# VGLoic/kzg-poly-commit-exploration

Hardware: AMD Instinct MI355X
Metric: g1_msm_commitments_per_sec_degree_2^20 (higher is better)
Workload: dtype i32 digits (Fp: 13 signed radix-2^30 digits, Montgomery 2^390; Fr: 8 x u32, Montgomery 2^256)

## Files before the change

kzg_poly_commit_exploration_amd/csrc/api.hip:

```cpp
#include <hip/hip_runtime.h>
#include <sys/random.h>

#include <algorithm>
#include <atomic>
#include <cerrno>
#include <chrono>
#include <condition_variable>
#include <cstdio>
#include <cstdlib>
#include <cstring>
#include <deque>
#include <functional>
#include <mutex>
#include <new>
#include <string>
#include <thread>
#include <vector>

#include "../../include/kzg_mi355x.h"
#include "engine.h"
#include "host_field.hpp"
#include "host_fr.hpp"
#include "fr30_host.hpp"
#include "host_pairing.hpp"
// ... 91 lines not shown
        DevBuf& b = buf[i];
        int rc = KZG_OK;
        if (!bytes && !b.p) {
            rc = b.reserve(ctx, 256);
            b.cap = 0;
        } else {
            rc = b.reserve(ctx, bytes);
        }
        *out = b.p;
        return rc;
    }
};

struct SlotQueue {
    hipStream_t stream = nullptr;
    hipStream_t end = nullptr;
    hipEvent_t ev[8] = {};
    hipEvent_t done = nullptr;
    hipEvent_t sorted_ev = nullptr, accum_ev = nullptr;
    hipEvent_t cmb_ev[2] = {};
    hipEvent_t cells_ev = nullptr;
    hipEvent_t upload_ev = nullptr;
    SlotQueue() = default;
    SlotQueue(const SlotQueue&) = delete;
    SlotQueue& operator=(const SlotQueue&) = delete;
    ~SlotQueue() {
        for (hipEvent_t e : {ev[0], ev[1], ev[2], ev[3], ev[4], ev[5], ev[6], ev[7], cmb_ev[0], cmb_ev[1], cells_ev, upload_ev, done, sorted_ev, accum_ev})
            if (e) hipEventDestroy(e);
    }
};

struct Slot : SlotQueue {
    DevBuf cnt, offs, block_sums, pairs, sorted, buckets;
    DevBuf part_a, part_b;
    DevBuf pair_scratch;
    DevBuf heavy_ws;
    DevBuf arena;
    PinnedBuf fin{PinnedBuf::Mapped};
    DevBuf stage;
    DevBuf q;
    DevBuf chunk, block;
    PinnedBuf small{PinnedBuf::Mapped};
    PinnedBuf bsmall{PinnedBuf::Mapped};
    std::vector<uint32_t> open_ys;
    PinnedBuf roots{PinnedBuf::Staged};
    PinnedBuf pvals{PinnedBuf::Mapped};
    DevBuf pblock;
    std::vector<uint32_t> pts_ys;
    size_t pts_nq = 0;
    PinnedBuf ctab{PinnedBuf::Staged};
    PinnedBuf cvals{PinnedBuf::Mapped};
    DevBuf cpart, cin;
    size_t cmb_t = 0;
    float combine_ms = 0;
    PinnedBuf stab{PinnedBuf::Staged}, ssel{PinnedBuf::Staged};
    PinnedBuf svals{PinnedBuf::Mapped};
    DevBuf sg;
    std::vector<uint32_t> sets_vmap;
    DevBuf lag_part;
    DevBuf gp_in, gp_z, gp_part;
    PinnedBuf gp_flags{PinnedBuf::Mapped};
    DevBuf cpoly, cagg;
    SlotKind kind = SLOT_IDLE;
    size_t job_n = 0;
    uint32_t job_batch = 1;
    uint32_t open_y[8] = {};
// ... 60 lines not shown
        if (_e != hipSuccess) {                                                                     \
            (ctx)->last_error = std::string(#expr) + ": " + hipGetErrorString(_e);                  \
            return KZG_ERR_HIP;                                                                     \
        }                                                                                           \
    } while (0)

int hip_fail(kzg_ctx* ctx, const char* what, hipError_t e) {
    ctx->last_error = std::string(what) + ": " + hipGetErrorString(e);
    return KZG_ERR_HIP;
}

struct TmpStream {
    hipStream_t s = nullptr;
    ~TmpStream() { if (s) hipStreamDestroy(s); }
};

int sync_unlocked(kzg_ctx* ctx, std::unique_lock<std::mutex>& lk, hipStream_t st, const char* what) {
    lk.unlock();
    const hipError_t e = hipStreamSynchronize(st);
    lk.lock();
    return e == hipSuccess ? KZG_OK : hip_fail(ctx, what, e);
}
constexpr const char* kCopyCoeffs = "hipMemcpyAsync (coefficients)";
int copy_unlocked(kzg_ctx* ctx, std::unique_lock<std::mutex>& lk, hipStream_t st, void* dst, const void* src, size_t bytes,
                  hipMemcpyKind kind, const char* what) {
    if (!bytes) return KZG_OK;
    lk.unlock();
    const hipError_t e = hipMemcpyAsync(dst, src, bytes, kind, st);
    lk.lock();
    return e == hipSuccess ? KZG_OK : hip_fail(ctx, what, e);
}

void free_slot_msm(Slot& s) {
    for (DevBuf* b : {&s.cnt, &s.offs, &s.block_sums, &s.pairs, &s.sorted, &s.buckets, &s.part_a, &s.part_b, &s.pair_scratch,
                      &s.heavy_ws, &s.arena})
        b->reset();
    s.fin.reset();
}

int create_stream(kzg_ctx* ctx, hipStream_t* out, bool high) {
    int least = 0, greatest = 0;
    HIP_TRY(ctx, hipDeviceGetStreamPriorityRange(&least, &greatest));
    const char* v = std::getenv("KZG_STREAM_PRIORITIES");
    const bool prio = !(v && v[0] == '0');
    HIP_TRY(ctx, hipStreamCreateWithPriority(out, hipStreamNonBlocking, prio ? (high ? greatest : least) : 0));
    return KZG_OK;
}

int ensure_slot_basics(kzg_ctx* ctx, Slot& s) {
    if (s.stream) return KZG_OK;
    if (!ctx->front_stream) {
        int rc = create_stream(ctx, &ctx->front_stream, false);
        if (rc) return rc;
    }
    if (!ctx->upload_stream) HIP_TRY(ctx, hipStreamCreateWithFlags(&ctx->upload_stream, hipStreamNonBlocking));
    for (auto& e : s.ev)
        if (!e) HIP_TRY(ctx, hipEventCreate(&e));
    if (!s.upload_ev) HIP_TRY(ctx, hipEventCreateWithFlags(&s.upload_ev, hipEventDisableTiming));
    s.stream = s.end = ctx->front_stream;
    if (!s.done) HIP_TRY(ctx, hipEventCreateWithFlags(&s.done, hipEventDisableTiming));
    return s.small.reserve(ctx, 64 * 4);
}

int upload_unlocked(kzg_ctx* ctx, std::unique_lock<std::mutex>& lk, Slot& s, void* dst, const void* src, size_t bytes) {
    if (!bytes) return KZG_OK;
    int rc = copy_unlocked(ctx, lk, ctx->upload_stream, dst, src, bytes, hipMemcpyHostToDevice, kCopyCoeffs);
    if (rc) return rc;
// ... 60 lines not shown
            ctx->last_error = "injected allocation failure (KZG_TEST_FAIL_SLOT_ALLOC)";
            return KZG_ERR_HIP;
        }
    }
    if (!ctx->heavy_stream) {
        int rc = create_stream(ctx, &ctx->heavy_stream, true);
        if (rc) return rc;
    }
    if (!ctx->tail_stream) {
        int rc = create_stream(ctx, &ctx->tail_stream, false);
        if (rc) return rc;
    }
    const MsmConfig cfg = ctx->cfg;
    if (ctx->max_batch > sort_max_batch(cfg)) ctx->max_batch = sort_max_batch(cfg);
    const size_t B = ctx->max_batch;
    const size_t pairs = (size_t)cfg.max_digits * ctx->n * B;
    for (int i = 0; i < kNumSlots; i++) {
        Slot& s = ctx->slots[i];
        {
            int rcb = ensure_slot_basics(ctx, s);
            if (rcb) return rcb;
        }
        if (!s.sorted_ev) {
            HIP_TRY(ctx, hipEventCreateWithFlags(&s.sorted_ev, hipEventDisableTiming));
            HIP_TRY(ctx, hipEventCreateWithFlags(&s.accum_ev, hipEventDisableTiming));
        }
        free_slot_msm(s);
        int rc = s.cnt.reserve(ctx, (size_t)sort_count_entries((uint32_t)B, cfg) * 4 + 64);
        if (rc == KZG_OK) rc = s.offs.reserve(ctx, ((size_t)cfg.nb * B + 1) * 4);
        if (rc == KZG_OK) rc = s.block_sums.reserve(ctx, (size_t)sort_workspace_words() * 4);
        if (rc) return rc;
        HIP_TRY(ctx, hipMemset(s.block_sums.p, 0, (size_t)sort_workspace_zero_words() * 4));
        rc = s.pairs.reserve(ctx, (pairs ? pairs : 1) * 8);
        if (rc == KZG_OK) rc = s.sorted.reserve(ctx, (pairs ? pairs : 1) * 4);
        if (rc == KZG_OK) rc = s.buckets.reserve(ctx, (size_t)cfg.nb * B * kXyzzBytes);
        if (rc == KZG_OK) rc = s.part_a.reserve(ctx, (size_t)kMaxAccumLanes * kXyzzBytes);
        if (rc == KZG_OK) rc = s.part_b.reserve(ctx, (size_t)kMaxAccumLanes * kXyzzBytes);
        if (rc == KZG_OK) rc = s.pair_scratch.reserve(ctx, accumulate_pair_scratch_bytes(pairs));
        if (rc == KZG_OK) rc = s.heavy_ws.reserve(ctx, heavy_workspace_bytes());
        if (rc == KZG_OK) rc = s.arena.reserve(ctx, ctx->arena_records * B * kXyzzBytes);
        if (rc == KZG_OK) rc = s.fin.reserve(ctx, ctx->final_records * B * kXyzzBytes);
        if (rc) return rc;
        s.kind = SLOT_IDLE;
    }
    ctx->slots_ready = true;
    return KZG_OK;
}

int build_tables(kzg_ctx* ctx, hipStream_t st, void* d_xyzz_tmp, void* d_prefix) {
    const size_t n = ctx->n;
    for (uint32_t j = 1; j < ctx->cfg.W; j++) {
        char* prev = (char*)ctx->table.p + (size_t)(j - 1) * n * kAffineBytes;
        char* next = (char*)ctx->table.p + (size_t)j * n * kAffineBytes;
        launch_table_window(st, prev, (uint32_t)n, ctx->cfg.level_bits, d_xyzz_tmp, d_prefix, next);
    }
    HIP_TRY(ctx, hipGetLastError());
    HIP_TRY(ctx, hipStreamSynchronize(st));
    return KZG_OK;
}

int drain_all(kzg_ctx* ctx) {
    for (hipStream_t st : {ctx->upload_stream, ctx->front_stream, ctx->heavy_stream, ctx->tail_stream})
        if (st) HIP_TRY(ctx, hipStreamSynchronize(st));
    return KZG_OK;
}

// ... 10 lines not shown
    ctx->srs_gen++;
    ctx->n = 0;
    return KZG_OK;
}

int srs_prepare(kzg_ctx* ctx, size_t n) {
    if (n == 0 || n > 0x7fffffffu / 32) return KZG_ERR_INVALID_ARG;
    int rc = srs_release(ctx);
    if (rc) return rc;
    size_t free_b = 0, total_b = 0;
    HIP_TRY(ctx, hipMemGetInfo(&free_b, &total_b));
    size_t budget = (size_t)((double)free_b * 0.6);
    if (const char* v = std::getenv("KZG_TABLE_GB")) budget = (size_t)(std::strtod(v, nullptr) * 1073741824.0);
    MsmConfig cfg = choose_msm_config(n, budget);
    if ((size_t)cfg.W * n >= 0x80000000ull) return KZG_ERR_INVALID_ARG;
    ctx->cfg = cfg;
    return ctx->table.reserve(ctx, (size_t)cfg.W * n * kAffineBytes);
}

struct MsmBasis {
    const void* table;
    uint32_t stride;
};
int enqueue_msm(kzg_ctx* ctx, Slot& s, const uint32_t* d_scalars, int is_mont, size_t n, int ev_base,
                uint32_t batch = 1, uint64_t stride = 0, const MsmBasis* basis = nullptr) {
    const MsmConfig cfg = ctx->cfg;
    const void* table = basis ? basis->table : ctx->table.p;
    const uint32_t table_stride = basis ? basis->stride : (uint32_t)ctx->n;
    const uint32_t nbt = cfg.nb * batch;
    hipStream_t st = s.stream;
    s.end = st;
    if (s.timing) HIP_TRY(ctx, hipEventRecord(s.ev[ev_base], st));
    const bool header_zeroed = launch_bucket_sort(st, d_scalars, is_mont, (uint32_t)n, batch, stride, table_stride, cfg, s.cnt.dev(),
                       s.block_sums.dev(), s.pairs.dev<uint64_t>(), s.offs.dev(), s.sorted.dev(), (uint32_t*)s.heavy_ws.p);
    if (s.timing) {
        HIP_TRY(ctx, hipEventRecord(s.ev[ev_base + 1], st));
        HIP_TRY(ctx, hipEventRecord(s.ev[ev_base + 2], st));
    }
    bool alone = true;
    for (const auto& other : ctx->slots) alone = alone && (&other == &s || other.kind == SLOT_IDLE);
    const uint64_t max_refs = (uint64_t)n * cfg.max_digits * batch;
    const uint32_t lanes = accumulate_lanes(max_refs, alone);
    const ReducePlan& P = ctx->plan;
    const uint32_t R = 1u << P.hi_bits, C = 1u << P.lo_bits, B = batch;
    char* row = (char*)s.arena.p;
    char* col = row + (size_t)R * B * kXyzzBytes;
    char* fin = (char*)s.fin.d;
    const uint32_t rl = 1u << P.row_lo, rh = 1u << P.row_hi, cl = 1u << P.col_lo, ch = 1u << P.col_hi;
    const TreeSumDesc stage1[2] = {
        {s.buckets.p, row, B * R, C, C, 1, B * R, 0},
        {s.buckets.p, col, B * C, R, 1, C, C, (uint64_t)cfg.nb}};
    const TreeSumDesc stage2[4] = {
        {row, fin + (size_t)P.off_r2row * B * kXyzzBytes, B * rh, rl, rl, 1, rh, R},
        {row, fin + (size_t)P.off_c2row * B * kXyzzBytes, B * rl, rh, 1, rl, rl, R},
        {col, fin + (size_t)P.off_r2col * B * kXyzzBytes, B * ch, cl, cl, 1, ch, C},
        {col, fin + (size_t)P.off_c2col * B * kXyzzBytes, B * cl, ch, 1, cl, cl, C}};
    if (!header_zeroed) HIP_TRY(ctx, hipMemsetAsync(s.heavy_ws.p, 0, kHeavyHeaderBytes, st));
    if (max_refs <= kTinyRefs && !ctx->small_msm_off) {
        if (s.timing) HIP_TRY(ctx, hipEventRecord(s.ev[ev_base + 3], st));
        launch_small_msm(st, table, s.sorted.dev(), s.offs.dev(), nbt, lanes, max_refs, s.buckets.p, s.part_a.p, s.part_b.p,
                         s.heavy_ws.p, s.small.dev() + 26, stage1, stage2, ctx->small_lds_bytes);
        if (s.timing) HIP_TRY(ctx, hipEventRecord(s.ev[ev_base + 4], st));
    } else {
        const bool hand_over = !alone;
        hipStream_t hs = hand_over ? ctx->heavy_stream : st;
        if (hand_over) {
            HIP_TRY(ctx, hipEventRecord(s.sorted_ev, st));
// ... 6658 lines not shown
```

kzg_poly_commit_exploration_amd/csrc/engine.h:

```cpp
#pragma once
#include <hip/hip_runtime.h>
#include <stddef.h>
#include <stdint.h>

namespace kzg {

constexpr size_t kAffineBytes = 128;
constexpr size_t kAffineU4 = kAffineBytes / 16;
constexpr size_t kXyzzBytes = 256;
constexpr size_t kXyzzU4 = kXyzzBytes / 16;
constexpr size_t kXyzzWords64 = kXyzzBytes / 8;

enum : uint32_t { kRecodeWindows = 0, kRecodeNaf = 1 };
struct MsmConfig {
    uint32_t recode;
    uint32_t c;
    uint32_t W;
    uint32_t level_bits;
    uint32_t nb;
    uint32_t max_digits;
};

MsmConfig choose_msm_config(size_t n_points, size_t table_budget_bytes);

constexpr uint32_t kTinyRefs = 65536;
__host__ __device__ inline uint32_t accumulate_min_seg(uint64_t refs) { return refs <= kTinyRefs ? 4u : 8u; }
__host__ __device__ inline uint32_t accumulate_seg_len(uint32_t M, uint32_t lanes) {
    uint32_t L = (M + lanes - 1) / lanes;
    const uint32_t lo = accumulate_min_seg(M);
    return L < lo ? lo : L;
}

constexpr size_t kHeavyHeaderBytes = 1024;
uint32_t sort_count_entries(uint32_t max_batch, MsmConfig cfg);
uint32_t sort_max_batch(MsmConfig cfg);
uint32_t sort_workspace_words();
uint32_t sort_workspace_zero_words();
bool launch_bucket_sort(hipStream_t s, const uint32_t* d_scalars, int scalars_are_mont, uint32_t n, uint32_t batch,
                        uint64_t stride, uint32_t table_stride, MsmConfig cfg, uint32_t* d_cnt,
                        uint32_t* d_ws, uint64_t* d_pairs, uint32_t* d_offs, uint32_t* d_sorted, uint32_t* d_header);
constexpr uint32_t kMaxAccumLanes = 262144 + 64;
uint32_t accumulate_lanes(uint64_t max_refs, bool alone = false);
size_t accumulate_pair_scratch_bytes(uint64_t max_refs);
void launch_bucket_accumulate(hipStream_t s, const void* d_table, const uint32_t* d_sorted, const uint32_t* d_offs,
                              uint32_t nb, uint32_t lanes, void* d_buckets ,
                              void* d_part_a, void* d_part_b, uint32_t lds_reserve_bytes, void* d_pair_scratch,
                              uint64_t max_refs, void* d_clock = nullptr );
constexpr size_t kAccumClockOffset = 768;
size_t heavy_workspace_bytes();
void launch_bucket_finalize(hipStream_t s, const uint32_t* d_offs, uint32_t nb, uint32_t lanes, const void* d_part_a,
                            const void* d_part_b, void* d_buckets, void* d_heavy_ws,
                            uint32_t* d_refs_out , uint32_t group = 1);
uint32_t finalize_group_size(uint32_t nb);
struct TreeSumDesc;
uint32_t small_msm_lds_bytes();
const void* small_msm_kernel();
void launch_small_msm(hipStream_t s, const void* d_table, const uint32_t* d_sorted, const uint32_t* d_offs, uint32_t nb,
                      uint32_t lanes, uint64_t max_refs, void* d_buckets, void* d_part_a, void* d_part_b, void* d_heavy_ws,
                      uint32_t* d_refs_out, const TreeSumDesc* stage1 , const TreeSumDesc* stage2 ,
                      uint32_t lds_bytes);
struct TreeSumDesc {
    const void* in;
    void* out;
    uint32_t groups, len;
    uint64_t gstride, estride;
    uint32_t inner;
    uint64_t ostride;
};
void launch_tree_sums(hipStream_t s, const TreeSumDesc* descs, uint32_t count, bool dense = false, bool alone = true);
void launch_tree_sums_two_stage(hipStream_t s, const TreeSumDesc* stage1, uint32_t count1, const TreeSumDesc* stage2,
                                uint32_t count2, uint32_t* d_sync, bool alone);

void launch_jacobian_to_affine(hipStream_t s, const void* d_jac, uint32_t n, void* d_affine_out,
// ... 257 lines not shown
```

kzg_poly_commit_exploration_amd/csrc/msm_sort.hip:

```cpp
#include <cstdlib>
#include <cstring>

#include "engine.h"
#include "fr30.hip.h"

namespace kzg {

typedef uint32_t u32;
#ifndef KZG_DEV
#define KZG_DEV __device__ __forceinline__
#endif

static uint32_t ilog2(uint32_t v) {
    uint32_t b = 0;
    while ((1u << b) < v) b++;
    return b;
}

MsmConfig choose_msm_config(size_t n, size_t table_budget_bytes) {
    const char* force_mode = std::getenv("KZG_MSM_RECODE");
    const char* force_c = std::getenv("KZG_MSM_C");
    const uint32_t fc = force_c ? (uint32_t)std::strtoul(force_c, nullptr, 10) : 0u;
    const bool naf = force_mode && !std::strcmp(force_mode, "naf") && n * 255ull < 0x80000000ull &&
                     (double)n * 255.0 * (double)kAffineBytes <= (double)table_budget_bytes;
    uint32_t best_c = 8;
    const uint32_t best_mode = naf ? kRecodeNaf : kRecodeWindows;
    double best = 1e300;
    for (uint32_t c = 8; c <= (naf ? 21u : 20u); c++) {
        if (fc >= 8 && fc <= (naf ? 21u : 20u) && c != fc) continue;
        if (!naf && !fc && 254u - c * ((255 + c - 1) / c - 1) < 4u) continue;
        double cost = naf ? (double)n * (255.0 / (c + 1) + 0.5) + 8.0 * (double)(1u << (c - 2))
                          : (double)n * ((255 + c - 1) / c) + 20.0 * (double)(1u << (c - 1));
        if (cost < best) {
            best = cost;
            best_c = c;
        }
    }
    MsmConfig cfg;
    cfg.recode = best_mode;
    cfg.c = best_c;
    if (best_mode == kRecodeNaf) {
        cfg.W = 255;
        cfg.level_bits = 1;
        cfg.nb = 1u << (best_c - 2);
        cfg.max_digits = (255 + best_c - 1) / best_c + 1;
    } else {
        cfg.W = (255 + best_c - 1) / best_c;
        cfg.level_bits = best_c;
        cfg.nb = 1u << (best_c - 1);
        cfg.max_digits = cfg.W;
    }
    return cfg;
}

KZG_DEV bool load_scalar(const uint32_t* d_scalars, uint64_t i, int is_mont, u32 k[8]) {
    const uint4* p = reinterpret_cast<const uint4*>(d_scalars) + 2 * (size_t)i;
    const uint4 lo = p[0], hi = p[1];
    const uint32_t in[8] = {lo.x, lo.y, lo.z, lo.w, hi.x, hi.y, hi.z, hi.w};
    const Fr30 d = fr30_from_limbs_raw(in);
    const Fr30 v = is_mont ? fr30_mul(d, fr30_small(1 << 14)) : fr30_mul(d, fr30_const_one270());
    return fr30_abs_to_limbs(v, k);
}

template <class F>
KZG_DEV void for_each_window_digit(u32 k[8], uint32_t c, uint32_t W, F&& f) {
    const u32 mask = (1u << c) - 1u;
    const u32 half = 1u << (c - 1);
    u32 carry = 0;
    for (uint32_t j = 0; j < W; j++) {
        u32 v = (k[0] & mask) + carry;
#pragma unroll
        for (int t = 0; t < 7; t++) k[t] = (k[t] >> c) | (k[t + 1] << (32 - c));
        k[7] >>= c;
        bool neg = v > half;
        u32 mag = neg ? (mask + 1u - v) : v;
        carry = neg ? 1u : 0u;
        if (mag) f(j, mag - 1u, neg);
    }
}

template <class F>
KZG_DEV void for_each_naf_digit(const u32 k[8], uint32_t c, F&& f) {
    const u32 mask = (1u << c) - 1u;
    const u32 half = 1u << (c - 1);
    u32 carry = 0;
    uint32_t p = 0;
#pragma unroll
    for (int t = 0; t < 8; t++) {
        const uint64_t win = ((uint64_t)(t < 7 ? k[t + 1] : 0u) << 32) | k[t];
        while (p < 32) {
            u32 x = (u32)(win >> p);
            if (carry) x = ~x;
            uint32_t z = x ? (uint32_t)__builtin_ctz(x) : 32u;
            if (z >= 32u - p) {
                p = 32;
                break;
            }
            p += z;
            u32 v = ((u32)(win >> p) & mask) + carry;
            const bool neg = v > half;
            const u32 mag = neg ? (mask + 1u - v) : v;
            carry = neg ? 1u : 0u;
            f(32u * (uint32_t)t + p, (mag - 1u) >> 1, neg);
            p += c;
        }
        p -= 32;
    }
}

template <class F>
KZG_DEV void for_each_digit(u32 k[8], MsmConfig cfg, F&& f) {
    if (cfg.recode == kRecodeNaf) for_each_naf_digit(k, cfg.c, f);
    else for_each_window_digit(k, cfg.c, cfg.W, f);
}

constexpr int kSortBlock = 256;
constexpr int kRecodeBlock = 1024;
#ifndef KZG_SORT_TILES
#define KZG_SORT_TILES 512
#endif
constexpr uint32_t kMaxTiles = KZG_SORT_TILES;
constexpr int kMaxCoarse = 2048;
constexpr int kFineMax = 256;

struct SortGeom {
    uint32_t tile;
    uint32_t tiles;
    uint32_t fine_bits;
    uint32_t coarse_bins;
    bool packed;
};

constexpr uint32_t kPackedFineBits = 7, kPackedIndexBits = 24;
static uint32_t sort_fine_bits(MsmConfig cfg, bool packed) {
    const uint32_t bits = ilog2(cfg.nb), most = packed ? kPackedFineBits : 8u;
    return bits < most ? bits : most;
}
static bool sort_packed_buckets(uint32_t nb_total, MsmConfig cfg);

static bool sort_packed_buckets(uint32_t nb_total, MsmConfig cfg) { return (nb_total >> sort_fine_bits(cfg, true)) <= (uint32_t)kMaxCoarse; }

static SortGeom sort_geometry(uint64_t total, uint32_t nb_total, MsmConfig cfg, uint32_t table_stride) {
    SortGeom g;
    static const bool allow_packed = [] { const char* v = std::getenv("KZG_SORT_PACKED"); return !(v && v[0] == '0'); }();
    g.packed = allow_packed && sort_packed_buckets(nb_total, cfg) && (uint64_t)cfg.W * table_stride <= (1ull << kPackedIndexBits);
    uint32_t tile = (uint32_t)((total + kMaxTiles - 1) / kMaxTiles);
    tile = ((tile + kSortBlock - 1) / kSortBlock) * kSortBlock;
    if (tile < (uint32_t)kSortBlock) tile = kSortBlock;
    g.tile = tile;
    g.tiles = (uint32_t)((total + tile - 1) / tile);
    g.fine_bits = sort_fine_bits(cfg, g.packed);
    g.coarse_bins = nb_total >> g.fine_bits;
    return g;
}

uint32_t sort_max_batch(MsmConfig cfg) {
    uint32_t fine_bits = sort_fine_bits(cfg, false);
    uint32_t b = (uint32_t)kMaxCoarse / (cfg.nb >> fine_bits);
    return b < 1 ? 1 : b;
}

uint32_t sort_count_entries(uint32_t max_batch, MsmConfig cfg) {
    uint32_t bins = 0;
    for (uint32_t b = 1; b <= max_batch; b++) {
        const uint32_t nbt = cfg.nb * b;
        const uint32_t q = nbt >> sort_fine_bits(cfg, sort_packed_buckets(nbt, cfg));
        if (q > bins) bins = q;
    }
    return bins * (kMaxTiles + 1u);
}

struct BatchGeom {
    uint32_t n;
    uint32_t batch;
    uint64_t stride;
    uint32_t nb;
};

__global__ void __launch_bounds__(kRecodeBlock) k_sort_count(const uint32_t* __restrict__ d_scalars, int is_mont,
                                                           BatchGeom bg, MsmConfig cfg, uint32_t tile,
                                                           uint32_t fine_bits, uint32_t coarse_bins,
                                                           uint32_t* __restrict__ d_cnt, uint32_t* __restrict__ d_binfill ,
                                                           uint32_t* __restrict__ d_header) {
    __shared__ u32 s_hist[kMaxCoarse];
    if (blockIdx.x == 0 && threadIdx.x < kHeavyHeaderBytes / 4) d_header[threadIdx.x] = 0;
    for (uint32_t q = threadIdx.x; q < coarse_bins; q += kRecodeBlock) s_hist[q] = 0;
    __syncthreads();
    const uint64_t base = (uint64_t)blockIdx.x * tile;
    const uint64_t total = (uint64_t)bg.n * bg.batch;
    for (uint32_t off = threadIdx.x; off < tile; off += kRecodeBlock) {
        uint64_t g = base + off;
        if (g >= total) break;
        uint32_t p = (uint32_t)(g / bg.n);
        uint32_t i = (uint32_t)(g - (uint64_t)p * bg.n);
        u32 k[8];
        (void)load_scalar(d_scalars, p * bg.stride + i, is_mont, k);
        const u32 pb = p * bg.nb;
        for_each_digit(k, cfg, [&](uint32_t, u32 bkt, bool) { atomicAdd(&s_hist[(pb + bkt) >> fine_bits], 1u); });
    }
    __syncthreads();
    for (uint32_t q = threadIdx.x; q < coarse_bins; q += kRecodeBlock) {
        const u32 c = s_hist[q];
        d_cnt[(size_t)blockIdx.x * coarse_bins + q] = c ? atomicAdd(&d_binfill[q], c) : 0u;
    }
}

template <int N>
__device__ __forceinline__ u32 block_exclusive_scan_n(u32 v, u32* lds, u32& total);
__device__ __forceinline__ u32 block_exclusive_scan_256(u32 v, u32* lds, u32& total);

constexpr uint32_t kFineMaxChunks = 4096;
constexpr uint32_t kFineLocal = 16;
constexpr uint32_t kWsBinStart = 0;
constexpr uint32_t kWsPrefix = kMaxCoarse + 8;
constexpr uint32_t kWsBinFill = 2 * kMaxCoarse + 32;
constexpr uint32_t kWsTable = 3 * kMaxCoarse + 64;
uint32_t sort_workspace_words() { return kWsTable + kFineMaxChunks * (uint32_t)kFineMax + 64; }
uint32_t sort_workspace_zero_words() { return kWsTable; }

template <int BLOCK>
KZG_DEV void spread_tile_cursors(uint32_t coarse_bins, const uint32_t* __restrict__ d_cnt, const uint32_t* __restrict__ d_binfill,
                                 uint32_t ch, uint32_t* __restrict__ d_binstart, uint32_t* __restrict__ d_prefix,
                                 uint32_t* __restrict__ d_total, u32* s_cur , u32* s_scan ) {
    const uint32_t t = threadIdx.x;
    constexpr uint32_t kStripes = kMaxCoarse / BLOCK;
    u32 below[kStripes], all[kStripes];
#pragma unroll
    for (uint32_t s = 0; s < kStripes; s++) {
        const uint32_t q = t + s * BLOCK;
        all[s] = q < coarse_bins ? d_binfill[q] : 0u;
        below[s] = q < coarse_bins ? d_cnt[(size_t)blockIdx.x * coarse_bins + q] : 0u;
    }
    u32 carry = 0, chunk_carry = 0;
#pragma unroll
    for (uint32_t s = 0; s < kStripes; s++) {
        if (s * BLOCK >= coarse_bins) break;
        const uint32_t q = t + s * BLOCK;
        u32 stripe_total;
        const u32 start = carry + block_exclusive_scan_n<BLOCK>(all[s], s_scan, stripe_total);
        __syncthreads();
        if (q < coarse_bins) s_cur[q] = start + below[s];
        if (blockIdx.x == 0) {
            const u32 nch = q < coarse_bins ? (all[s] + ch - 1) / ch : 0u;
            u32 chunk_total;
            const u32 cstart = chunk_carry + block_exclusive_scan_n<BLOCK>(nch, s_scan, chunk_total);
            __syncthreads();
            if (q < coarse_bins) {
                d_binstart[q] = start;
                d_prefix[q] = cstart;
            }
            chunk_carry += chunk_total;
        }
        carry += stripe_total;
    }
    if (blockIdx.x == 0 && t == 0) {
        d_binstart[coarse_bins] = carry;
        d_prefix[coarse_bins] = chunk_carry;
        *d_total = carry;
    }
    __syncthreads();
}

__global__ void __launch_bounds__(kRecodeBlock) k_sort_spread(const uint32_t* __restrict__ d_scalars, int is_mont,
                                                            BatchGeom bg, uint32_t table_stride, MsmConfig cfg,
                                                            uint32_t tile, uint32_t tiles, uint32_t fine_bits,
                                                            uint32_t coarse_bins, const uint32_t* __restrict__ d_cnt ,
                                                            const uint32_t* __restrict__ d_binfill ,
                                                            uint32_t ch, uint32_t* __restrict__ d_binstart,
                                                            uint32_t* __restrict__ d_prefix, uint32_t* __restrict__ d_total,
                                                            uint64_t* __restrict__ d_pairs, int packed) {
    __shared__ u32 s_cur[kMaxCoarse];
    __shared__ u32 s_scan[kRecodeBlock];
    spread_tile_cursors<kRecodeBlock>(coarse_bins, d_cnt, d_binfill, ch, d_binstart, d_prefix, d_total, s_cur, s_scan);
    const uint64_t base = (uint64_t)blockIdx.x * tile;
    const uint64_t total = (uint64_t)bg.n * bg.batch;
    const u32 fine_mask = (1u << fine_bits) - 1u;
    for (uint32_t off = threadIdx.x; off < tile; off += kRecodeBlock) {
        uint64_t g = base + off;
        if (g >= total) break;
        uint32_t p = (uint32_t)(g / bg.n);
        uint32_t i = (uint32_t)(g - (uint64_t)p * bg.n);
        u32 k[8];
        const bool flip = load_scalar(d_scalars, p * bg.stride + i, is_mont, k);
        const u32 pb = p * bg.nb;
        for_each_digit(k, cfg, [&](uint32_t j, u32 bkt, bool neg) {
            u32 b = pb + bkt;
            u32 pos = atomicAdd(&s_cur[b >> fine_bits], 1u);
            u32 ref = (j * table_stride + i) | ((neg != flip) ? 0x80000000u : 0u);
            if (packed) reinterpret_cast<u32*>(d_pairs)[pos] = ref | ((b & fine_mask) << kPackedIndexBits);
            else d_pairs[pos] = ((uint64_t)(b & fine_mask) << 32) | ref;
        });
    }
}

constexpr int kStageBlock = 512;
constexpr uint32_t kStageSlots = 7680;

template <int BLOCK>
KZG_DEV u32 block_exclusive_scan_fast(u32 v, u32* s_wave , u32& total) {
    const uint32_t t = threadIdx.x, lane = t & 63u, w = t >> 6;
    u32 incl = v;
#pragma unroll
    for (uint32_t off = 1; off < 64; off <<= 1) {
        const u32 up = __shfl_up(incl, off, 64);
        if (lane >= off) incl += up;
    }
    if (lane == 63) s_wave[w] = incl;
    __syncthreads();
    u32 base = 0, all = 0;
#pragma unroll
    for (uint32_t i = 0; i < BLOCK / 64; i++) {
        const u32 x = s_wave[i];
        if (i < w) base += x;
        all += x;
    }
    __syncthreads();
    total = all;
    return base + incl - v;
}

__global__ void __launch_bounds__(kStageBlock) k_sort_spread_staged(const uint32_t* __restrict__ d_scalars, int is_mont,
                                                                  BatchGeom bg, uint32_t table_stride, MsmConfig cfg,
                                                                  uint32_t tile, uint32_t fine_bits, uint32_t coarse_bins,
                                                                  const uint32_t* __restrict__ d_cnt, const uint32_t* __restrict__ d_binfill,
                                                                  uint32_t ch, uint32_t* __restrict__ d_binstart,
                                                                  uint32_t* __restrict__ d_prefix, uint32_t* __restrict__ d_total,
                                                                  uint32_t* __restrict__ d_pairs32) {
    __shared__ u32 s_cur[kMaxCoarse];
    __shared__ u32 s_cnt[kMaxCoarse];
    __shared__ u32 s_gd[kMaxCoarse];
    __shared__ u32 s_scan[kStageBlock];
    __shared__ u32 s_stage[kStageSlots];
    __shared__ uint16_t s_sbin[kStageSlots];
    spread_tile_cursors<kStageBlock>(coarse_bins, d_cnt, d_binfill, ch, d_binstart, d_prefix, d_total, s_cur, s_scan);
    const uint32_t t = threadIdx.x;
    const uint64_t base = (uint64_t)blockIdx.x * tile;
    const uint64_t total = (uint64_t)bg.n * bg.batch;
    const u32 fine_mask = (1u << fine_bits) - 1u;
    const uint32_t per_round = kStageSlots / cfg.max_digits < (uint32_t)kStageBlock ? kStageSlots / cfg.max_digits : (uint32_t)kStageBlock;
    constexpr uint32_t kBinsPerLane = kMaxCoarse / kStageBlock;
    for (uint32_t r0 = 0; r0 < tile; r0 += per_round) {
        for (uint32_t q = t; q < coarse_bins; q += kStageBlock) s_cnt[q] = 0;
        __syncthreads();
        const uint32_t off = r0 + t;
        const uint64_t g = base + off;
        const bool valid = t < per_round && off < tile && g < total;
        u32 k[8];
        bool flip = false;
        uint32_t i = 0;
        u32 pb = 0;
        if (valid) {
            const uint32_t p = (uint32_t)(g / bg.n);
            i = (uint32_t)(g - (uint64_t)p * bg.n);
            pb = p * bg.nb;
            flip = load_scalar(d_scalars, p * bg.stride + i, is_mont, k);
            u32 k1[8];
#pragma unroll
            for (int w = 0; w < 8; w++) k1[w] = k[w];
            for_each_digit(k1, cfg, [&](uint32_t, u32 bkt, bool) { atomicAdd(&s_cnt[(pb + bkt) >> fine_bits], 1u); });
        }
        __syncthreads();
        u32 mine[kBinsPerLane], sum = 0;
#pragma unroll
        for (uint32_t e = 0; e < kBinsPerLane; e++) {
            const uint32_t q = t * kBinsPerLane + e;
            mine[e] = q < coarse_bins ? s_cnt[q] : 0u;
            sum += mine[e];
        }
        u32 round_total;
        u32 run = block_exclusive_scan_fast<kStageBlock>(sum, s_scan, round_total);
#pragma unroll
        for (uint32_t e = 0; e < kBinsPerLane; e++) {
            const uint32_t q = t * kBinsPerLane + e;
            if (q < coarse_bins) {
                const u32 cur = s_cur[q];
                s_gd[q] = cur - run;
                s_cur[q] = cur + mine[e];
                s_cnt[q] = run;
            }
            run += mine[e];
        }
        __syncthreads();
        if (valid) {
            for_each_digit(k, cfg, [&](uint32_t j, u32 bkt, bool neg) {
                const u32 b = pb + bkt, bin = b >> fine_bits;
                const u32 slot = atomicAdd(&s_cnt[bin], 1u);
                s_stage[slot] = (j * table_stride + i) | ((neg != flip) ? 0x80000000u : 0u) | ((b & fine_mask) << kPackedIndexBits);
                s_sbin[slot] = (uint16_t)bin;
            });
        }
        __syncthreads();
        for (uint32_t e = t; e < round_total; e += kStageBlock) d_pairs32[s_gd[s_sbin[e]] + e] = s_stage[e];
    }
}


static uint32_t fine_chunk_len(uint64_t max_pairs) {
    static const uint64_t target = [] {
        const char* v = std::getenv("KZG_FINE_CHUNKS");
        uint64_t t = v ? std::strtoull(v, nullptr, 10) : 2048ull;
        return t < 1 ? 1ull : (t > 2048 ? 2048ull : t);
    }();
    uint64_t ch = (max_pairs + target - 1) / target;
    ch = (ch + 255) / 256 * 256;
    return (uint32_t)(ch < 4096 ? 4096 : ch);
}

struct FineChunk {
    uint32_t bin, beg, end, nch, j, base;
};
KZG_DEV bool locate_chunk(uint32_t k, const uint32_t* __restrict__ d_prefix, const uint32_t* __restrict__ d_binstart,
                          uint32_t coarse_bins, uint32_t ch, FineChunk& c) {
    if (k >= d_prefix[coarse_bins]) return false;
    uint32_t lo = 0, hi = coarse_bins;
    while (hi - lo > 1) {
        uint32_t mid = (lo + hi) >> 1;
        if (d_prefix[mid] <= k) lo = mid; else hi = mid;
// ... 176 lines not shown
    int t = threadIdx.x;
    lds[t] = v;
    __syncthreads();
    for (int off = 1; off < N; off <<= 1) {
        u32 add = t >= off ? lds[t - off] : 0u;
        __syncthreads();
        lds[t] += add;
        __syncthreads();
    }
    total = lds[N - 1];
    return lds[t] - v;
}
__device__ __forceinline__ u32 block_exclusive_scan_256(u32 v, u32* lds, u32& total) { return block_exclusive_scan_n<256>(v, lds, total); }

constexpr uint32_t kSmallSortScalars = 4096;
constexpr uint32_t kSmallSortBuckets = 4096;
constexpr int kSmallSortBlock = 1024;

__global__ void __launch_bounds__(kSmallSortBlock) k_sort_small(const uint32_t* __restrict__ d_scalars, int is_mont, uint32_t n,
                                                                uint32_t table_stride, MsmConfig cfg,
                                                                uint32_t* __restrict__ d_offs,
                                                                uint32_t* __restrict__ d_sorted,
                                                                uint32_t* __restrict__ d_header) {
    __shared__ u32 s_hist[kSmallSortBuckets];
    if (blockIdx.x == 0 && threadIdx.x < kHeavyHeaderBytes / 4) d_header[threadIdx.x] = 0;
    __shared__ u32 s_part[kSmallSortBlock];
    const uint32_t t = threadIdx.x;
    const uint32_t nb = cfg.nb;
    for (uint32_t b = t; b < nb; b += kSmallSortBlock) s_hist[b] = 0;
    __syncthreads();
    for (uint32_t i = t; i < n; i += kSmallSortBlock) {
        u32 k[8];
        (void)load_scalar(d_scalars, i, is_mont, k);
        for_each_digit(k, cfg, [&](uint32_t, u32 bkt, bool) { atomicAdd(&s_hist[bkt], 1u); });
    }
    __syncthreads();
    const uint32_t per = (nb + kSmallSortBlock - 1) / kSmallSortBlock;
    u32 local = 0;
    for (uint32_t q = 0; q < per; q++) {
        uint32_t b = t * per + q;
        if (b < nb) local += s_hist[b];
    }
    s_part[t] = local;
    __syncthreads();
    for (int off = 1; off < kSmallSortBlock; off <<= 1) {
        u32 add = t >= (uint32_t)off ? s_part[t - off] : 0u;
        __syncthreads();
        s_part[t] += add;
        __syncthreads();
    }
    u32 run = s_part[t] - local;
    for (uint32_t q = 0; q < per; q++) {
        uint32_t b = t * per + q;
        if (b < nb) {
            u32 c = s_hist[b];
            d_offs[b] = run;
            s_hist[b] = run;
            run += c;
        }
    }
    if (t == kSmallSortBlock - 1) d_offs[nb] = s_part[t];
    __syncthreads();
    const uint32_t b_lo = (uint32_t)((uint64_t)nb * blockIdx.x / gridDim.x), b_hi = (uint32_t)((uint64_t)nb * (blockIdx.x + 1) / gridDim.x);
    for (uint32_t i = t; i < n; i += kSmallSortBlock) {
        u32 k[8];
        const bool flip = load_scalar(d_scalars, i, is_mont, k);
        for_each_digit(k, cfg, [&](uint32_t j, u32 bkt, bool neg) {
            if (bkt >= b_lo && bkt < b_hi) {
                u32 pos = atomicAdd(&s_hist[bkt], 1u);
                d_sorted[pos] = (j * table_stride + i) | ((neg != flip) ? 0x80000000u : 0u);
            }
        });
    }
}

bool launch_bucket_sort(hipStream_t s, const uint32_t* d_scalars, int is_mont, uint32_t n, uint32_t batch,
                        uint64_t stride, uint32_t table_stride, MsmConfig cfg, uint32_t* d_cnt, uint32_t* d_ws,
                        uint64_t* d_pairs, uint32_t* d_offs, uint32_t* d_sorted, uint32_t* d_header) {
    if (n == 0 || batch == 0) return false;
    static const bool small_path = [] { const char* v = std::getenv("KZG_SMALL_SORT"); return !(v && v[0] == '0'); }();
    if (small_path && batch == 1 && n <= kSmallSortScalars && cfg.nb <= kSmallSortBuckets) {
        uint32_t groups = n / 256;
        groups = groups < 1 ? 1 : (groups > 8 ? 8 : groups);
        hipLaunchKernelGGL(k_sort_small, dim3(groups), dim3(kSmallSortBlock), 0, s, d_scalars, is_mont, n, table_stride, cfg, d_offs,
                           d_sorted, d_header);
        return true;
    }
    const uint32_t nb_total = cfg.nb * batch;
    SortGeom g = sort_geometry((uint64_t)n * batch, nb_total, cfg, table_stride);
    BatchGeom bg{n, batch, stride, cfg.nb};
    uint32_t* d_binstart = d_ws + kWsBinStart;
    uint32_t* d_prefix = d_ws + kWsPrefix;
    uint32_t* d_table = d_ws + kWsTable;
    uint32_t* d_total = d_offs + nb_total;
    const uint64_t max_pairs = (uint64_t)n * batch * cfg.max_digits;
    const uint32_t ch = fine_chunk_len(max_pairs);
    const uint32_t max_chunks = (uint32_t)((max_pairs + ch - 1) / ch) + g.coarse_bins;
    uint32_t* d_binfill = d_ws + kWsBinFill;
    hipLaunchKernelGGL(k_sort_count, dim3(g.tiles), dim3(kRecodeBlock), 0, s, d_scalars, is_mont, bg, cfg, g.tile,
                       g.fine_bits, g.coarse_bins, d_cnt, d_binfill, d_header);
    static const bool staged = [] { const char* v = std::getenv("KZG_SPREAD_STAGED"); return !(v && v[0] == '0'); }();
    if (g.packed && staged && cfg.max_digits <= kStageSlots)
        hipLaunchKernelGGL(k_sort_spread_staged, dim3(g.tiles), dim3(kStageBlock), 0, s, d_scalars, is_mont, bg, table_stride, cfg,
                           g.tile, g.fine_bits, g.coarse_bins, d_cnt, d_binfill, ch, d_binstart, d_prefix, d_total,
                           reinterpret_cast<uint32_t*>(d_pairs));
    else
        hipLaunchKernelGGL(k_sort_spread, dim3(g.tiles), dim3(kRecodeBlock), 0, s, d_scalars, is_mont, bg, table_stride, cfg,
                           g.tile, g.tiles, g.fine_bits, g.coarse_bins, d_cnt, d_binfill, ch, d_binstart, d_prefix, d_total, d_pairs,
                           g.packed ? 1 : 0);
    if (g.packed)
        hipLaunchKernelGGL(k_fine_count<true>, dim3(max_chunks), dim3(kSortBlock), 0, s, reinterpret_cast<const uint32_t*>(d_pairs),
                           d_binstart, g.fine_bits, g.coarse_bins, ch, d_prefix, d_table, d_binfill);
    else
        hipLaunchKernelGGL(k_fine_count<false>, dim3(max_chunks), dim3(kSortBlock), 0, s, d_pairs, d_binstart, g.fine_bits,
                           g.coarse_bins, ch, d_prefix, d_table, d_binfill);
    hipLaunchKernelGGL(k_fine_binscan, dim3(g.coarse_bins), dim3(kSortBlock), 0, s, d_binstart, g.fine_bits, d_prefix, d_table, d_offs);
    if (g.packed)
        hipLaunchKernelGGL(k_fine_scatter<true>, dim3(max_chunks), dim3(kSortBlock), 0, s, reinterpret_cast<const uint32_t*>(d_pairs),
                           d_binstart, g.fine_bits, g.coarse_bins, ch, d_prefix, d_table, d_offs, d_sorted);
    else
        hipLaunchKernelGGL(k_fine_scatter<false>, dim3(max_chunks), dim3(kSortBlock), 0, s, d_pairs, d_binstart, g.fine_bits,
                           g.coarse_bins, ch, d_prefix, d_table, d_offs, d_sorted);
    return true;
}

}
```

Baseline: 418.5.

## Cache recoded scalars between sort passes and specialize window digit extraction

The count kernel now stores each folded, sign-flipped scalar to a new per-slot buffer, and the spread kernels load it instead of reloading and re-running the Montgomery conversion. Window digit extraction gets compile-time-width specializations for common window sizes (15, 16, 17, 19), which replace the loop that shifts all eight limbs per digit. The recode block size is also halved. The cost is an extra 32 bytes per scalar of device memory plus one write and one read of it per MSM.

```diff
diff --git a/kzg_poly_commit_exploration_amd/csrc/api.hip b/kzg_poly_commit_exploration_amd/csrc/api.hip
--- a/kzg_poly_commit_exploration_amd/csrc/api.hip
+++ b/kzg_poly_commit_exploration_amd/csrc/api.hip
@@ -147,6 +147,7 @@
 
 struct Slot : SlotQueue {
     DevBuf cnt, offs, block_sums, pairs, sorted, buckets;
+    DevBuf recoded;
     DevBuf part_a, part_b;
     DevBuf pair_scratch;
     DevBuf heavy_ws;
@@ -273,7 +274,7 @@
 }
 
 void free_slot_msm(Slot& s) {
-    for (DevBuf* b : {&s.cnt, &s.offs, &s.block_sums, &s.pairs, &s.sorted, &s.buckets, &s.part_a, &s.part_b, &s.pair_scratch,
+    for (DevBuf* b : {&s.cnt, &s.offs, &s.block_sums, &s.pairs, &s.recoded, &s.sorted, &s.buckets, &s.part_a, &s.part_b, &s.pair_scratch,
                       &s.heavy_ws, &s.arena})
         b->reset();
     s.fin.reset();
@@ -400,6 +401,7 @@
         if (rc) return rc;
         HIP_TRY(ctx, hipMemset(s.block_sums.p, 0, (size_t)sort_workspace_zero_words() * 4));
         rc = s.pairs.reserve(ctx, (pairs ? pairs : 1) * 8);
+        if (rc == KZG_OK) rc = s.recoded.reserve(ctx, (ctx->n * B ? ctx->n * B : 1) * 32);
         if (rc == KZG_OK) rc = s.sorted.reserve(ctx, (pairs ? pairs : 1) * 4);
         if (rc == KZG_OK) rc = s.buckets.reserve(ctx, (size_t)cfg.nb * B * kXyzzBytes);
         if (rc == KZG_OK) rc = s.part_a.reserve(ctx, (size_t)kMaxAccumLanes * kXyzzBytes);
@@ -476,7 +478,7 @@
     s.end = st;
     if (s.timing) HIP_TRY(ctx, hipEventRecord(s.ev[ev_base], st));
     const bool header_zeroed = launch_bucket_sort(st, d_scalars, is_mont, (uint32_t)n, batch, stride, table_stride, cfg, s.cnt.dev(),
-                       s.block_sums.dev(), s.pairs.dev<uint64_t>(), s.offs.dev(), s.sorted.dev(), (uint32_t*)s.heavy_ws.p);
+                       s.block_sums.dev(), s.pairs.dev<uint64_t>(), s.recoded.dev(), s.offs.dev(), s.sorted.dev(), (uint32_t*)s.heavy_ws.p);
     if (s.timing) {
         HIP_TRY(ctx, hipEventRecord(s.ev[ev_base + 1], st));
         HIP_TRY(ctx, hipEventRecord(s.ev[ev_base + 2], st));
diff --git a/kzg_poly_commit_exploration_amd/csrc/engine.h b/kzg_poly_commit_exploration_amd/csrc/engine.h
--- a/kzg_poly_commit_exploration_amd/csrc/engine.h
+++ b/kzg_poly_commit_exploration_amd/csrc/engine.h
@@ -38,7 +38,8 @@
 uint32_t sort_workspace_zero_words();
 bool launch_bucket_sort(hipStream_t s, const uint32_t* d_scalars, int scalars_are_mont, uint32_t n, uint32_t batch,
                         uint64_t stride, uint32_t table_stride, MsmConfig cfg, uint32_t* d_cnt,
-                        uint32_t* d_ws, uint64_t* d_pairs, uint32_t* d_offs, uint32_t* d_sorted, uint32_t* d_header);
+                        uint32_t* d_ws, uint64_t* d_pairs, uint32_t* d_recoded, uint32_t* d_offs, uint32_t* d_sorted,
+                        uint32_t* d_header);
 constexpr uint32_t kMaxAccumLanes = 262144 + 64;
 uint32_t accumulate_lanes(uint64_t max_refs, bool alone = false);
 size_t accumulate_pair_scratch_bytes(uint64_t max_refs);
diff --git a/kzg_poly_commit_exploration_amd/csrc/msm_recode.h b/kzg_poly_commit_exploration_amd/csrc/msm_recode.h
--- /dev/null
+++ b/kzg_poly_commit_exploration_amd/csrc/msm_recode.h
@@ -0,0 +1,94 @@
+#pragma once
+#include <stdint.h>
+
+#include <utility>
+
+#include "fr30.hip.h"
+
+namespace kzg {
+
+KZG_HD bool recode_fold(const uint32_t in[8], int is_mont, uint32_t k[8]) {
+    const Fr30 d = fr30_from_limbs_raw(in);
+    const Fr30 v = is_mont ? fr30_mul(d, fr30_small(1 << 14)) : fr30_mul(d, fr30_const_one270());
+    return fr30_abs_to_limbs(v, k);
+}
+
+KZG_HD void recode_pack(uint32_t k[8], bool flip) { k[7] |= flip ? 0x80000000u : 0u; }
+KZG_HD bool recode_unpack(uint32_t k[8]) {
+    const bool flip = (k[7] >> 31) != 0;
+    k[7] &= 0x7fffffffu;
+    return flip;
+}
+
+template <class F>
+KZG_HD void for_each_window_digit(uint32_t k[8], uint32_t c, uint32_t W, F&& f) {
+    const uint32_t mask = (1u << c) - 1u;
+    const uint32_t half = 1u << (c - 1);
+    uint32_t carry = 0;
+    for (uint32_t j = 0; j < W; j++) {
+        uint32_t v = (k[0] & mask) + carry;
+#pragma unroll
+        for (int t = 0; t < 7; t++) k[t] = (k[t] >> c) | (k[t + 1] << (32 - c));
+        k[7] >>= c;
+        bool neg = v > half;
+        uint32_t mag = neg ? (mask + 1u - v) : v;
+        carry = neg ? 1u : 0u;
+        if (mag) f(j, mag - 1u, neg);
+    }
+}
+
+template <uint32_t C, uint32_t J, class F>
+KZG_HD void window_digit_fixed(const uint32_t k[8], uint32_t& carry, F& f) {
+    constexpr uint32_t mask = (1u << C) - 1u;
+    constexpr uint32_t half = 1u << (C - 1);
+    constexpr uint32_t w = (J * C) >> 5, s = (J * C) & 31u;
+    constexpr bool straddles = s + C > 32u && w < 7u;
+    uint32_t bits = k[w] >> s;
+    if constexpr (straddles) bits |= k[w + 1u] << (32u - s);
+    const uint32_t v = (bits & mask) + carry;
+    const bool neg = v > half;
+    const uint32_t mag = neg ? (mask + 1u - v) : v;
+    carry = neg ? 1u : 0u;
+    if (mag) f(J, mag - 1u, neg);
+}
+template <uint32_t C, class F, uint32_t... J>
+KZG_HD void window_digits_fixed(const uint32_t k[8], F& f, std::integer_sequence<uint32_t, J...>) {
+    uint32_t carry = 0;
+    (window_digit_fixed<C, J>(k, carry, f), ...);
+}
+template <uint32_t C, class F>
+KZG_HD void for_each_window_digit_fixed(const uint32_t k[8], F&& f) {
+    static_assert(C >= 2 && C <= 31, "a window is cut out of two adjacent words");
+    window_digits_fixed<C>(k, f, std::make_integer_sequence<uint32_t, (255 + C - 1) / C>());
+}
+
+template <class F>
+KZG_HD void for_each_naf_digit(const uint32_t k[8], uint32_t c, F&& f) {
+    const uint32_t mask = (1u << c) - 1u;
+    const uint32_t half = 1u << (c - 1);
+    uint32_t carry = 0;
+    uint32_t p = 0;
+#pragma unroll
+    for (int t = 0; t < 8; t++) {
+        const uint64_t win = ((uint64_t)(t < 7 ? k[t + 1] : 0u) << 32) | k[t];
+        while (p < 32) {
+            uint32_t x = (uint32_t)(win >> p);
+            if (carry) x = ~x;
+            uint32_t z = x ? (uint32_t)__builtin_ctz(x) : 32u;
+            if (z >= 32u - p) {
+                p = 32;
+                break;
+            }
+            p += z;
+            uint32_t v = ((uint32_t)(win >> p) & mask) + carry;
+            const bool neg = v > half;
+            const uint32_t mag = neg ? (mask + 1u - v) : v;
+            carry = neg ? 1u : 0u;
+            f(32u * (uint32_t)t + p, (mag - 1u) >> 1, neg);
+            p += c;
+        }
+        p -= 32;
+    }
+}
+
+}
diff --git a/kzg_poly_commit_exploration_amd/csrc/msm_sort.hip b/kzg_poly_commit_exploration_amd/csrc/msm_sort.hip
--- a/kzg_poly_commit_exploration_amd/csrc/msm_sort.hip
+++ b/kzg_poly_commit_exploration_amd/csrc/msm_sort.hip
@@ -1,8 +1,10 @@
 #include <cstdlib>
 #include <cstring>
+#include <type_traits>
 
 #include "engine.h"
 #include "fr30.hip.h"
+#include "msm_recode.h"
 
 namespace kzg {
 
@@ -57,65 +59,40 @@
     const uint4* p = reinterpret_cast<const uint4*>(d_scalars) + 2 * (size_t)i;
     const uint4 lo = p[0], hi = p[1];
     const uint32_t in[8] = {lo.x, lo.y, lo.z, lo.w, hi.x, hi.y, hi.z, hi.w};
-    const Fr30 d = fr30_from_limbs_raw(in);
-    const Fr30 v = is_mont ? fr30_mul(d, fr30_small(1 << 14)) : fr30_mul(d, fr30_const_one270());
-    return fr30_abs_to_limbs(v, k);
-}
-
-template <class F>
-KZG_DEV void for_each_window_digit(u32 k[8], uint32_t c, uint32_t W, F&& f) {
-    const u32 mask = (1u << c) - 1u;
-    const u32 half = 1u << (c - 1);
-    u32 carry = 0;
-    for (uint32_t j = 0; j < W; j++) {
-        u32 v = (k[0] & mask) + carry;
-#pragma unroll
-        for (int t = 0; t < 7; t++) k[t] = (k[t] >> c) | (k[t + 1] << (32 - c));
-        k[7] >>= c;
-        bool neg = v > half;
-        u32 mag = neg ? (mask + 1u - v) : v;
-        carry = neg ? 1u : 0u;
-        if (mag) f(j, mag - 1u, neg);
-    }
-}
-
-template <class F>
-KZG_DEV void for_each_naf_digit(const u32 k[8], uint32_t c, F&& f) {
-    const u32 mask = (1u << c) - 1u;
-    const u32 half = 1u << (c - 1);
-    u32 carry = 0;
-    uint32_t p = 0;
-#pragma unroll
-    for (int t = 0; t < 8; t++) {
-        const uint64_t win = ((uint64_t)(t < 7 ? k[t + 1] : 0u) << 32) | k[t];
-        while (p < 32) {
-            u32 x = (u32)(win >> p);
-            if (carry) x = ~x;
-            uint32_t z = x ? (uint32_t)__builtin_ctz(x) : 32u;
-            if (z >= 32u - p) {
-                p = 32;
-                break;
-            }
-            p += z;
-            u32 v = ((u32)(win >> p) & mask) + carry;
-            const bool neg = v > half;
-            const u32 mag = neg ? (mask + 1u - v) : v;
-            carry = neg ? 1u : 0u;
-            f(32u * (uint32_t)t + p, (mag - 1u) >> 1, neg);
-            p += c;
-        }
-        p -= 32;
-    }
-}
-
-template <class F>
-KZG_DEV void for_each_digit(u32 k[8], MsmConfig cfg, F&& f) {
-    if (cfg.recode == kRecodeNaf) for_each_naf_digit(k, cfg.c, f);
-    else for_each_window_digit(k, cfg.c, cfg.W, f);
+    return recode_fold(in, is_mont, k);
+}
+
+KZG_DEV void store_recoded(uint32_t* d_recoded, uint64_t g, const u32 k[8], bool flip) {
+    uint4* p = reinterpret_cast<uint4*>(d_recoded) + 2 * (size_t)g;
+    p[0] = make_uint4(k[0], k[1], k[2], k[3]);
+    p[1] = make_uint4(k[4], k[5], k[6], k[7] | (flip ? 0x80000000u : 0u));
+}
+KZG_DEV bool load_recoded(const uint32_t* d_recoded, uint64_t g, u32 k[8]) {
+    const uint4* p = reinterpret_cast<const uint4*>(d_recoded) + 2 * (size_t)g;
+    const uint4 lo = p[0], hi = p[1];
+    k[0] = lo.x, k[1] = lo.y, k[2] = lo.z, k[3] = lo.w, k[4] = hi.x, k[5] = hi.y, k[6] = hi.z, k[7] = hi.w;
+    return recode_unpack(k);
+}
+
+template <uint32_t C, class F>
+KZG_DEV void for_each_digit(const u32 k[8], MsmConfig cfg, F&& f) {
+    if constexpr (C != 0) {
+        for_each_window_digit_fixed<C>(k, f);
+    } else if (cfg.recode == kRecodeNaf) {
+        for_each_naf_digit(k, cfg.c, f);
+    } else {
+        u32 t[8];
+#pragma unroll
+        for (int w = 0; w < 8; w++) t[w] = k[w];
+        for_each_window_digit(t, cfg.c, cfg.W, f);
+    }
+}
+static uint32_t fixed_width(MsmConfig cfg) {
+    return cfg.recode == kRecodeWindows && (cfg.c == 15 || cfg.c == 16 || cfg.c == 17 || cfg.c == 19) ? cfg.c : 0u;
 }
 
 constexpr int kSortBlock = 256;
-constexpr int kRecodeBlock = 1024;
+constexpr int kRecodeBlock = 512;
 #ifndef KZG_SORT_TILES
 #define KZG_SORT_TILES 512
 #endif
@@ -177,9 +154,11 @@
     uint32_t nb;
 };
 
+template <uint32_t C>
 __global__ void __launch_bounds__(kRecodeBlock) k_sort_count(const uint32_t* __restrict__ d_scalars, int is_mont,
                                                            BatchGeom bg, MsmConfig cfg, uint32_t tile,
                                                            uint32_t fine_bits, uint32_t coarse_bins,
+                                                           uint32_t* __restrict__ d_recoded ,
                                                            uint32_t* __restrict__ d_cnt, uint32_t* __restrict__ d_binfill ,
                                                            uint32_t* __restrict__ d_header) {
     __shared__ u32 s_hist[kMaxCoarse];
@@ -194,9 +173,10 @@
         uint32_t p = (uint32_t)(g / bg.n);
         uint32_t i = (uint32_t)(g - (uint64_t)p * bg.n);
         u32 k[8];
-        (void)load_scalar(d_scalars, p * bg.stride + i, is_mont, k);
+        const bool flip = load_scalar(d_scalars, p * bg.stride + i, is_mont, k);
+        store_recoded(d_recoded, g, k, flip);
         const u32 pb = p * bg.nb;
-        for_each_digit(k, cfg, [&](uint32_t, u32 bkt, bool) { atomicAdd(&s_hist[(pb + bkt) >> fine_bits], 1u); });
+        for_each_digit<C>(k, cfg, [&](uint32_t, u32 bkt, bool) { atomicAdd(&s_hist[(pb + bkt) >> fine_bits], 1u); });
     }
     __syncthreads();
     for (uint32_t q = threadIdx.x; q < coarse_bins; q += kRecodeBlock) {
@@ -261,7 +241,8 @@
     __syncthreads();
 }
 
-__global__ void __launch_bounds__(kRecodeBlock) k_sort_spread(const uint32_t* __restrict__ d_scalars, int is_mont,
+template <uint32_t C>
+__global__ void __launch_bounds__(kRecodeBlock) k_sort_spread(const uint32_t* __restrict__ d_recoded,
                                                             BatchGeom bg, uint32_t table_stride, MsmConfig cfg,
                                                             uint32_t tile, uint32_t tiles, uint32_t fine_bits,
                                                             uint32_t coarse_bins, const uint32_t* __restrict__ d_cnt ,
@@ -281,9 +262,9 @@
         uint32_t p = (uint32_t)(g / bg.n);
         uint32_t i = (uint32_t)(g - (uint64_t)p * bg.n);
         u32 k[8];
-        const bool flip = load_scalar(d_scalars, p * bg.stride + i, is_mont, k);
+        const bool flip = load_recoded(d_recoded, g, k);
         const u32 pb = p * bg.nb;
-        for_each_digit(k, cfg, [&](uint32_t j, u32 bkt, bool neg) {
+        for_each_digit<C>(k, cfg, [&](uint32_t j, u32 bkt, bool neg) {
             u32 b = pb + bkt;
             u32 pos = atomicAdd(&s_cur[b >> fine_bits], 1u);
             u32 ref = (j * table_stride + i) | ((neg != flip) ? 0x80000000u : 0u);
@@ -319,7 +300,8 @@
     return base + incl - v;
 }
 
-__global__ void __launch_bounds__(kStageBlock) k_sort_spread_staged(const uint32_t* __restrict__ d_scalars, int is_mont,
+template <uint32_t C>
+__global__ void __launch_bounds__(kStageBlock) k_sort_spread_staged(const uint32_t* __restrict__ d_recoded,
                                                                   BatchGeom bg, uint32_t table_stride, MsmConfig cfg,
                                                                   uint32_t tile, uint32_t fine_bits, uint32_t coarse_bins,
                                                                   const uint32_t* __restrict__ d_cnt, const uint32_t* __restrict__ d_binfill,
@@ -353,11 +335,8 @@
             const uint32_t p = (uint32_t)(g / bg.n);
             i = (uint32_t)(g - (uint64_t)p * bg.n);
             pb = p * bg.nb;
-            flip = load_scalar(d_scalars, p * bg.stride + i, is_mont, k);
-            u32 k1[8];
-#pragma unroll
-            for (int w = 0; w < 8; w++) k1[w] = k[w];
-            for_each_digit(k1, cfg, [&](uint32_t, u32 bkt, bool) { atomicAdd(&s_cnt[(pb + bkt) >> fine_bits], 1u); });
+            flip = load_recoded(d_recoded, g, k);
+            for_each_digit<C>(k, cfg, [&](uint32_t, u32 bkt, bool) { atomicAdd(&s_cnt[(pb + bkt) >> fine_bits], 1u); });
         }
         __syncthreads();
         u32 mine[kBinsPerLane], sum = 0;
@@ -382,7 +361,7 @@
         }
         __syncthreads();
         if (valid) {
-            for_each_digit(k, cfg, [&](uint32_t j, u32 bkt, bool neg) {
+            for_each_digit<C>(k, cfg, [&](uint32_t j, u32 bkt, bool neg) {
                 const u32 b = pb + bkt, bin = b >> fine_bits;
                 const u32 slot = atomicAdd(&s_cnt[bin], 1u);
                 s_stage[slot] = (j * table_stride + i) | ((neg != flip) ? 0x80000000u : 0u) | ((b & fine_mask) << kPackedIndexBits);
@@ -625,7 +604,7 @@
     for (uint32_t i = t; i < n; i += kSmallSortBlock) {
         u32 k[8];
         (void)load_scalar(d_scalars, i, is_mont, k);
-        for_each_digit(k, cfg, [&](uint32_t, u32 bkt, bool) { atomicAdd(&s_hist[bkt], 1u); });
+        for_each_digit<0>(k, cfg, [&](uint32_t, u32 bkt, bool) { atomicAdd(&s_hist[bkt], 1u); });
     }
     __syncthreads();
     const uint32_t per = (nb + kSmallSortBlock - 1) / kSmallSortBlock;
@@ -658,7 +637,7 @@
     for (uint32_t i = t; i < n; i += kSmallSortBlock) {
         u32 k[8];
         const bool flip = load_scalar(d_scalars, i, is_mont, k);
-        for_each_digit(k, cfg, [&](uint32_t j, u32 bkt, bool neg) {
+        for_each_digit<0>(k, cfg, [&](uint32_t j, u32 bkt, bool neg) {
             if (bkt >= b_lo && bkt < b_hi) {
                 u32 pos = atomicAdd(&s_hist[bkt], 1u);
                 d_sorted[pos] = (j * table_stride + i) | ((neg != flip) ? 0x80000000u : 0u);
@@ -669,7 +648,7 @@
 
 bool launch_bucket_sort(hipStream_t s, const uint32_t* d_scalars, int is_mont, uint32_t n, uint32_t batch,
                         uint64_t stride, uint32_t table_stride, MsmConfig cfg, uint32_t* d_cnt, uint32_t* d_ws,
-                        uint64_t* d_pairs, uint32_t* d_offs, uint32_t* d_sorted, uint32_t* d_header) {
+                        uint64_t* d_pairs, uint32_t* d_recoded, uint32_t* d_offs, uint32_t* d_sorted, uint32_t* d_header) {
     if (n == 0 || batch == 0) return false;
     static const bool small_path = [] { const char* v = std::getenv("KZG_SMALL_SORT"); return !(v && v[0] == '0'); }();
     if (small_path && batch == 1 && n <= kSmallSortScalars && cfg.nb <= kSmallSortBuckets) {
@@ -690,17 +669,28 @@
     const uint32_t ch = fine_chunk_len(max_pairs);
     const uint32_t max_chunks = (uint32_t)((max_pairs + ch - 1) / ch) + g.coarse_bins;
     uint32_t* d_binfill = d_ws + kWsBinFill;
-    hipLaunchKernelGGL(k_sort_count, dim3(g.tiles), dim3(kRecodeBlock), 0, s, d_scalars, is_mont, bg, cfg, g.tile,
-                       g.fine_bits, g.coarse_bins, d_cnt, d_binfill, d_header);
     static const bool staged = [] { const char* v = std::getenv("KZG_SPREAD_STAGED"); return !(v && v[0] == '0'); }();
-    if (g.packed && staged && cfg.max_digits <= kStageSlots)
-        hipLaunchKernelGGL(k_sort_spread_staged, dim3(g.tiles), dim3(kStageBlock), 0, s, d_scalars, is_mont, bg, table_stride, cfg,
-                           g.tile, g.fine_bits, g.coarse_bins, d_cnt, d_binfill, ch, d_binstart, d_prefix, d_total,
-                           reinterpret_cast<uint32_t*>(d_pairs));
-    else
-        hipLaunchKernelGGL(k_sort_spread, dim3(g.tiles), dim3(kRecodeBlock), 0, s, d_scalars, is_mont, bg, table_stride, cfg,
-                           g.tile, g.tiles, g.fine_bits, g.coarse_bins, d_cnt, d_binfill, ch, d_binstart, d_prefix, d_total, d_pairs,
-                           g.packed ? 1 : 0);
+    const bool use_staged = g.packed && staged && cfg.max_digits <= kStageSlots;
+    auto recode = [&](auto width) {
+        constexpr uint32_t C = decltype(width)::value;
+        hipLaunchKernelGGL(k_sort_count<C>, dim3(g.tiles), dim3(kRecodeBlock), 0, s, d_scalars, is_mont, bg, cfg, g.tile, g.fine_bits,
+                           g.coarse_bins, d_recoded, d_cnt, d_binfill, d_header);
+        if (use_staged)
+            hipLaunchKernelGGL(k_sort_spread_staged<C>, dim3(g.tiles), dim3(kStageBlock), 0, s, d_recoded, bg, table_stride, cfg,
+                               g.tile, g.fine_bits, g.coarse_bins, d_cnt, d_binfill, ch, d_binstart, d_prefix, d_total,
+                               reinterpret_cast<uint32_t*>(d_pairs));
+        else
+            hipLaunchKernelGGL(k_sort_spread<C>, dim3(g.tiles), dim3(kRecodeBlock), 0, s, d_recoded, bg, table_stride, cfg, g.tile,
+                               g.tiles, g.fine_bits, g.coarse_bins, d_cnt, d_binfill, ch, d_binstart, d_prefix, d_total, d_pairs,
+                               g.packed ? 1 : 0);
+    };
+    switch (fixed_width(cfg)) {
+        case 15: recode(std::integral_constant<uint32_t, 15>()); break;
+        case 16: recode(std::integral_constant<uint32_t, 16>()); break;
+        case 17: recode(std::integral_constant<uint32_t, 17>()); break;
+        case 19: recode(std::integral_constant<uint32_t, 19>()); break;
+        default: recode(std::integral_constant<uint32_t, 0>()); break;
+    }
     if (g.packed)
         hipLaunchKernelGGL(k_fine_count<true>, dim3(max_chunks), dim3(kSortBlock), 0, s, reinterpret_cast<const uint32_t*>(d_pairs),
                            d_binstart, g.fine_bits, g.coarse_bins, ch, d_prefix, d_table, d_binfill);
```

After: 435.6, median of 6. +4.1%, better.
